# jhong93/vpd

Hardware: AMD Instinct MI355X
Metric: frame-crops/sec (VPD student train) (higher is better)
Workload: dtype bf16; 1 GPU; configs[1]: Diving48-shaped synthetic crops 128x128, ResNet-34 student (5-ch RGB+flow), emb_dim 128, sum-MSE + AdamW, batch=256 per GPU; global_batch=256, parallelism=dp1

## Files before the change

### include/vpd_hip.h

```cpp
#ifndef VPD_HIP_H
#define VPD_HIP_H
#include <stddef.h>
#ifdef __cplusplus
extern "C" {
#endif

typedef struct vpd_plan vpd_plan_t;

const char* vpd_last_error(void);
int vpd_abi_version(void);
const char* vpd_elem_dtype(void);

int vpd_plan_create(const char* arch, int c_in, int img_h, int img_w, int emb_dim, int motion,
                    int max_batch, int train, vpd_plan_t** out);
#define VPD_TRAIN_EARLY_BUCKET0 2
void vpd_plan_destroy(vpd_plan_t* plan);

int vpd_plan_num_tensors(const vpd_plan_t* plan);
int vpd_plan_tensor_info(const vpd_plan_t* plan, int i, int* kind, int* is_decoder, long long* offset,
                         long long* numel, int* ndim, int dims[4]);
long long vpd_plan_param_numel(const vpd_plan_t* plan);
int vpd_plan_num_bn(const vpd_plan_t* plan);
int vpd_plan_bn_info(const vpd_plan_t* plan, int i, int* channels, long long* rm_off, long long* rv_off);
long long vpd_plan_bn_numel(const vpd_plan_t* plan);
// ... 127 lines not shown
int vpd_graph_launch_eval(vpd_plan_t* plan, int n, void* stream);

int vpd_plan_sync_errors(vpd_plan_t* plan, void* workspace, void* stream, unsigned* count_out);

int vpd_plan_set_timing(vpd_plan_t* plan, int enable);
int vpd_plan_read_timing(vpd_plan_t* plan, double* out, int nclasses);

int vpd_op_conv2d(const void* x_bf16, const void* w_bf16, void* y_bf16, double* stats, int n, int xHp, int xWp,
                  int xC, int yHp, int yWp, int yC, int ypad, int Hs, int Ws, int osub, int oph, int opw, int istr,
                  int Kc, int Co, const int* tapset9, int accumulate, void* stream);
int vpd_op_conv_bm(int M, int Co);
int vpd_op_conv2d_ep(const void* x_bf16, const void* w_bf16, void* y_bf16, int n, int xHp, int xWp, int xC, int yHp, int yWp,
                     int yC, int ypad, int Hs, int Ws, int istr, int Kc, int Co, const int* tapset9, const float* ep_scale,
                     const float* ep_shift, const void* res_padded_bf16, int ep_relu, int accumulate,
                     const unsigned char* acc_mask, void* stream);
int vpd_op_conv2d_bnsums(const void* x_bf16, const void* w_bf16, void* y_bf16, const void* bst_z_bf16,
                         const unsigned char* bst_mask, double* rows, int n, int xHp, int xWp, int xC, int Hs, int Ws,
                         int Kc, int Co, const int* tapset9, int accumulate, void* stream);
int vpd_op_conv2d_bnsums2(const void* x_bf16, const void* w_bf16, void* y_bf16, const void* bst_z_bf16,
                          const unsigned char* bst_mask, double* rows, const void* bst_z2_bf16, double* rows2, int n, int xHp,
                          int xWp, int xC, int Hs, int Ws, int Kc, int Co, const int* tapset9, void* stream);
int vpd_op_conv2d_dispatch(int n, int xHp, int xWp, int xC, int yHp, int yWp, int yC, int ypad, int Hs, int Ws, int osub, int oph,
                           int opw, int istr, int Kc, int Co, const int* tapset9, int accumulate, int flags, int* out12);
int vpd_op_bn_forward(const void* z_bf16, const double* rows, const float* gamma, const float* beta, float* running_mean,
                      float* running_var, float* mean, float* rstd, float* scale, float* shift, const void* res_padded_bf16,
                      void* out_padded_bf16, unsigned char* mask_bits, int n, int H, int W, int C, int relu, float momentum,
                      float eps, void* stream);
int vpd_op_set_bn_frozen(int on);
int vpd_op_bn_forward2(const void* z_bf16, const double* rows, const float* gamma, const float* beta, float* running_mean,
                       float* running_var, float* mean, float* rstd, float* scale, float* shift, const void* z2_bf16,
                       const double* rows2, const float* gamma2, const float* beta2, float* running_mean2, float* running_var2,
                       float* mean2, float* rstd2, float* scale2, float* shift2, void* out_padded_bf16, unsigned char* mask_bits,
                       int n, int H, int W, int C, int relu, float momentum, float eps, void* stream);
int vpd_op_bn_finalize(double* rows, const float* gamma, const float* beta, float* running_mean, float* running_var, float* mean,
                       float* rstd, float* scale, float* shift, int count, int C, float momentum, float eps, void* stream);
int vpd_op_bn_apply(const void* z_bf16, const float* scale, const float* shift, const void* res_bf16, const float* rscale,
                    const float* rshift, int res_kind, void* out_padded_bf16, int n, int H, int W, int C, int relu, void* stream);
int vpd_op_bn_backward_apply(const void* dy_bf16, const void* z_bf16, const unsigned char* mask_bits, const double* rows,
                             const float* gamma, const float* mean, const float* rstd, void* dz_padded_bf16, float* dgamma,
                             float* dbeta, int n, int H, int W, int C, void* stream);
int vpd_op_bn_backward_apply2(const void* dy_bf16, const void* z_bf16, const unsigned char* mask_bits, const double* rows,
                              const float* gamma, const float* mean, const float* rstd, void* dz_padded_bf16, float* dgamma,
                              float* dbeta, const void* z2_bf16, const double* rows2, const float* gamma2, const float* mean2,
                              const float* rstd2, void* dz2_padded_bf16, float* dgamma2, float* dbeta2, int n, int H, int W, int C,
                              void* stream);
int vpd_op_conv1x1_bn(int mode, const void* x_padded, const void* w, int n, int H, int W, int istr, int Kc, int Co, double* rows,
// ... 76 lines not shown
```

### vpd_amd/_lib.py

```python
import ctypes as C
import os

_HERE = os.path.dirname(os.path.abspath(__file__))
LIB_PATH = os.environ.get("VPD_LIB_PATH") or os.path.join(_HERE, "libvpdhip.so")
LIB_PATH_F16 = os.environ.get("VPD_LIB_PATH_F16") or os.path.join(_HERE, "libvpdhip_f16.so")
ABI_VERSION = 5

c_int_p = C.POINTER(C.c_int)
c_ll_p = C.POINTER(C.c_longlong)
c_dbl_p = C.POINTER(C.c_double)
vp = C.c_void_p

SIGNATURES = {
    "vpd_last_error": (C.c_char_p, []),
    "vpd_abi_version": (C.c_int, []),
    "vpd_elem_dtype": (C.c_char_p, []),
    "vpd_plan_create": (C.c_int, [C.c_char_p, C.c_int, C.c_int, C.c_int, C.c_int, C.c_int, C.c_int, C.c_int,
                                  C.POINTER(vp)]),
    "vpd_plan_destroy": (None, [vp]),
    "vpd_plan_num_tensors": (C.c_int, [vp]),
    "vpd_plan_tensor_info": (C.c_int, [vp, C.c_int, c_int_p, c_int_p, c_ll_p, c_ll_p, c_int_p, c_int_p]),
    "vpd_plan_param_numel": (C.c_longlong, [vp]),
    "vpd_plan_num_bn": (C.c_int, [vp]),
    "vpd_plan_bn_info": (C.c_int, [vp, C.c_int, c_int_p, c_ll_p, c_ll_p]),
# ... 38 lines not shown
    "vpd_plan_grad_norm": (C.c_int, [vp, vp, C.c_longlong, C.c_double, vp, C.c_float, vp, vp, vp]),
    "vpd_adam_groups_bytes": (C.c_size_t, [C.c_int]),
    "vpd_adam_groups_init": (C.c_int, [vp, vp, c_ll_p, c_int_p, C.c_int, C.c_longlong, C.c_int, vp]),
    "vpd_adamw_step_groups": (C.c_int, [vp, vp, vp, vp, C.c_longlong, vp, c_dbl_p, c_dbl_p, C.c_int, C.c_double, C.c_double,
                                        C.c_double, C.c_int, C.c_float, vp, vp]),
    "vpd_plan_adamw_step_groups": (C.c_int, [vp, vp, vp, vp, vp, C.c_longlong, vp, c_dbl_p, c_dbl_p, C.c_int, C.c_double,
                                             C.c_double, C.c_double, C.c_int, vp, vp, vp]),
    "vpd_op_grad_accumulate": (C.c_int, [C.POINTER(vp), C.POINTER(vp), c_ll_p, C.c_int, C.c_int, vp]),
    "vpd_plan_grad_accum_numel": (C.c_longlong, [vp]),
    "vpd_plan_grad_accumulate": (C.c_int, [vp, vp, C.c_longlong, vp, C.c_int, vp, vp]),
    "vpd_plan_bucket_scratch_range": (C.c_int, [vp, C.c_int, C.POINTER(C.c_longlong), C.POINTER(C.c_longlong)]),
    "vpd_plan_grads_pending": (C.c_int, [vp]),
    "vpd_plan_materialize_grads": (C.c_int, [vp, vp, vp, vp]),
    "vpd_plan_set_bn_frozen": (C.c_int, [vp, C.c_int]),
    "vpd_plan_set_param_grads": (C.c_int, [vp, C.c_int]),
    "vpd_plan_set_timing": (C.c_int, [vp, C.c_int]),
    "vpd_plan_read_timing": (C.c_int, [vp, C.POINTER(C.c_double), C.c_int]),
    "vpd_op_conv2d": (C.c_int, [vp, vp, vp, vp] + [C.c_int] * 16 + [c_int_p, C.c_int, vp]),
    "vpd_op_conv_bm": (C.c_int, [C.c_int, C.c_int]),
    "vpd_op_conv2d_ep": (C.c_int, [vp, vp, vp] + [C.c_int] * 13 + [c_int_p, vp, vp, vp, C.c_int, C.c_int, vp, vp]),
    "vpd_op_conv2d_bnsums": (C.c_int, [vp] * 6 + [C.c_int] * 8 + [c_int_p, C.c_int, vp]),
    "vpd_op_conv2d_bnsums2": (C.c_int, [vp] * 8 + [C.c_int] * 8 + [c_int_p, vp]),
    "vpd_op_conv2d_dispatch": (C.c_int, [C.c_int] * 16 + [c_int_p, C.c_int, C.c_int, c_int_p]),
    "vpd_op_bn_forward": (C.c_int, [vp] * 13 + [C.c_int] * 5 + [C.c_float, C.c_float, vp]),
    "vpd_op_set_bn_frozen": (C.c_int, [C.c_int]),
    "vpd_op_bn_forward2": (C.c_int, [vp] * 22 + [C.c_int] * 5 + [C.c_float, C.c_float, vp]),
    "vpd_op_bn_finalize": (C.c_int, [vp] * 9 + [C.c_int, C.c_int, C.c_float, C.c_float, vp]),
    "vpd_op_bn_apply": (C.c_int, [vp] * 6 + [C.c_int, vp] + [C.c_int] * 5 + [vp]),
    "vpd_op_bn_backward_apply": (C.c_int, [vp] * 10 + [C.c_int] * 4 + [vp]),
    "vpd_op_bn_backward_apply2": (C.c_int, [vp] * 18 + [C.c_int] * 4 + [vp]),
    "vpd_op_conv1x1_bn": (C.c_int, [C.c_int, vp, vp] + [C.c_int] * 6 + [vp] * 5 + [C.c_float, C.c_float] + [vp] * 12),
    "vpd_op_conv1x1_bn2": (C.c_int, [C.c_int] + [vp] * 4 + [C.c_int] * 6 + [vp] * 18 + [C.c_float, C.c_float] + [vp] * 10),
    "vpd_op_conv1x1_bn_dispatch": (C.c_int, [C.c_int] * 6 + [c_int_p]),
    "vpd_op_stem_pool_forward": (C.c_int, [vp] * 5 + [C.c_int] * 5 + [vp]),
    "vpd_op_stem_dgrad": (C.c_int, [vp, vp, vp, C.c_int, C.c_int, C.c_int, C.c_int, vp]),
    "vpd_op_stem_pool_backward": (C.c_int, [vp] * 15 + [C.c_int] * 4 + [vp]),
    "vpd_op_bn_backward": (C.c_int, [vp] * 15 + [C.c_int] + [vp, vp] + [C.c_int] * 6 + [vp]),
    "vpd_op_bn_backward_pair": (C.c_int, [vp] * 20 + [C.c_int] * 4 + [vp]),
    "vpd_op_bn_backward_residency": (C.c_int, [C.c_int, C.c_int, C.c_int, c_int_p]),
    "vpd_op_avgpool": (C.c_int, [vp] + [C.c_int] * 5 + [vp, vp]),
    "vpd_op_avgpool_bwd": (C.c_int, [vp] + [C.c_int] * 4 + [vp, vp]),
    "vpd_op_sgemm": (C.c_int, [vp] * 4 + [C.c_int] * 6 + [vp]),
    "vpd_op_colsum": (C.c_int, [vp, C.c_int, C.c_int, vp, vp]),
    "vpd_op_relu_mask": (C.c_int, [vp, vp, C.c_longlong, vp]),
    "vpd_op_mse": (C.c_int, [vp, vp, C.c_longlong, vp, vp, vp, vp]),
    "vpd_op_wgrad": (C.c_int, [vp, vp, vp] + [C.c_int] * 13 + [c_int_p, vp, vp]),
# ... 71 lines not shown
```

### vpd_amd/csrc/conv_igemm.hip

```cpp
#include <stdlib.h>
#include <stdio.h>

#include <algorithm>
#include <vector>

#include "common.h"
#include "conv_epilogue.h"
#include "kernels.h"

static __device__ __forceinline__ void conv_take_alt(ConvParams& p, const ConvParams& p0, int& by) {
    if (p0.alt_w && by >= p0.alt_y0) {
        by -= p0.alt_y0;
        p.w = p0.alt_w; p.y = p0.alt_y; p.stats = p0.alt_stats; p.taps = p0.alt_taps;
        p.ep_scale = p0.alt_ep_scale; p.ep_shift = p0.alt_ep_shift; p.ep_relu = p0.alt_ep_relu; p.res = nullptr;
    }
}

static __device__ __forceinline__ int conv_pixel_base(const ConvParams& p, const ConvGeo& geo, int m) {
    const int HW = geo.Hs * geo.Ws;
    m = m < geo.M ? m : geo.M - 1;
    const int b = m / HW;
    const int r = m - b * HW;
    const int yy = r / geo.Ws;
    const int xx = r - yy * geo.Ws;
// ... 1280 lines not shown
    dim3 grid((p.M + BM - 1) / BM, p.Co / BN);
    size_t lds = ((size_t)(HALO2 ? 2 : 1) * HROWS + 2 * BN) * 64 * sizeof(bf16_t);
    const size_t red = (size_t)2 * 2 * BN * sizeof(float);
    if (lds < red) lds = red;
    ConvParams q = p;
    VPD_LAUNCH((conv3x3_halo_kernel<BM, BN, HROWS, HALO2>), grid, dim3(256), lds, stream, q, g);
    return hipGetLastError();
}

static bool halo_geom(const ConvParams& p, int BM, int hrows_max, HaloGeom* g) {
    const int W = p.Ws, H = p.Hs;
    if (BM % W != 0) return false;
    const int TR = BM / W;
    if (TR <= H) { if (H % TR != 0) return false; g->multi = 0; g->HR = TR + 2; }
    else { if (TR % H != 0) return false; g->multi = 1; g->HR = (TR / H) * (H + 2); }
    g->TR = TR;
    g->NHP = g->HR * (W + 2);
    g->total_pix = p.N * (H + 2) * (W + 2);
    if (W >= 8) { g->kmask = 7; g->kshift = 0; g->rowmask = 0; }
    else { g->kmask = 3; g->kshift = 2; g->rowmask = 1; }
    g->rH = 1.0f / (float)H; g->rW = 1.0f / (float)W; g->rWp = 1.0f / (float)(W + 2);
    g->rot = vpd_switches().pws_rot && p.Kc > 64 && conv_ep_mode(p) != 3;
    g->rnch = 1.0f / (float)(p.Kc / 64);
    return g->NHP <= hrows_max;
}

static bool halo_eligible(const ConvParams& p) {
    return p.taps.nr == 3 && p.taps.nc == 3 && p.istr == 1 && p.osub == 1 && p.oph == 0 && p.opw == 0 &&
           p.xC == p.Kc && p.xHp == p.Hs + 2 && p.xWp == p.Ws + 2 && p.taps.dy0 + 2 * p.taps.dys >= 0 &&
           p.taps.dy0 >= 0 && p.taps.dy0 <= 2 && p.taps.dx0 >= 0 && p.taps.dx0 <= 2 &&
           p.taps.dy0 + 2 * p.taps.dys <= 2 && p.taps.dx0 + 2 * p.taps.dxs >= 0 && p.taps.dx0 + 2 * p.taps.dxs <= 2;
}

template <int BM, int BN, int WM, int WN>
static hipError_t launch_cfg(const ConvParams& p, hipStream_t stream) {
    ConvParams q = p;
    const dim3 grid = conv_class_grid(q, BM, BN);
    const size_t lds = (size_t)2 * (BM + BN) * 64 * sizeof(bf16_t);
    switch (conv_ep_mode(q)) {
        case 0: VPD_LAUNCH((conv_igemm_kernel<BM, BN, WM, WN, 0>), grid, dim3(256), lds, stream, q); break;
        case 1: VPD_LAUNCH((conv_igemm_kernel<BM, BN, WM, WN, 1>), grid, dim3(256), lds, stream, q); break;
        case 2: VPD_LAUNCH((conv_igemm_kernel<BM, BN, WM, WN, 2>), grid, dim3(256), lds, stream, q); break;
        case 6: VPD_LAUNCH((conv_igemm_kernel<BM, BN, WM, WN, 6>), grid, dim3(256), lds, stream, q); break;
        case 7: VPD_LAUNCH((conv_igemm_kernel<BM, BN, WM, WN, 7>), grid, dim3(256), lds, stream, q); break;
        default: VPD_LAUNCH((conv_igemm_kernel<BM, BN, WM, WN, 3>), grid, dim3(256), lds, stream, q); break;
    }
// ... 63 lines not shown
    if (p.x2 || p.osub != 1) return false;
    if (p.yWp != p.Ws || p.yHp != p.Hs) return false;
    if (p.bst_z2) return p.accumulate && p.stats2 && (kc == 1 || kc == 2 || kc == 3 || kc == 6);
    if (kc == 0) {
        HaloGeom g2;
        return vpd_switches().dgrad_sums_l1 && !c64x2_geom(p, &g2);
    }
    return kc == 1 || kc == 2 || kc == 3 || kc == 6;
}

ConvDispatch vpd_conv_dispatch(const ConvParams& p, HaloGeom* g) {
    ConvDispatch d = {};
    d.mode = conv_ep_mode(p);
    d.kclass = vpd_conv_kernel_class(p, g);
    d.tiles_per_block = 1;
    const auto pws_form = [&](int bm, int bn, int hrows, int ns, int nmw, bool on) {
        d.bm = bm; d.bn = bn;
        d.pws = on && pws_enabled(p);
        if (!d.pws) return;
        const PwsGrid sg = pws_grid(p, bm, bn);
        d.tiles_per_block = (sg.MT + sg.lanes - 1) / sg.lanes;
        bool flip;
        d.geo = vpd_switches().pws_geo ? vpd_pws_geo_width(bm, bn, hrows, ns, nmw, p, *g, &flip) : 0;
    };
    switch (d.kclass) {
        case 0: {
            HaloGeom g2;
            d.c64x2 = c64x2_geom(p, &g2);
            if (d.c64x2) *g = g2;
            d.bm = d.c64x2 ? 256 : 128; d.bn = 64;
            const int ntiles = (p.M + d.bm - 1) / d.bm;
            int per;
            const int grid = persistent_grid(ntiles, &per);
            d.tiles_per_block = (ntiles + grid - 1) / grid;
            return d;
        }
        case 1: pws_form(256, 128, 352, PWS_NS_C1, 8, (p.M + 255) / 256 > pws_cu_count() / (p.Co / 128)); return d;
        case 2: pws_form(128, 128, 288, PWS_NS_C2, 4, true); return d;
        case 3: pws_form(128, 64, 288, PWS_NS_C3, 4, true); return d;
        case 6: pws_form(256, 64, 416, PWS_NS_C6, 4, true); return d;
        case 5: {
            d.bm = 128; d.bn = 64;
            const int grid = stem_grid(p);
            d.tiles_per_block = p.pool_y ? (p.N + grid - 1) / grid * (p.Hs * p.Ws / 128) : (p.M / 128 + grid - 1) / grid;
            return d;
        }
// ... 64 lines not shown
```

### vpd_amd/csrc/conv_pws.h

```cpp
#pragma once
#include <type_traits>

#include "common.h"
#include "conv_epilogue.h"

struct HaloGeom {
    int TR;
    int multi;
    int HR;
    int NHP;
    int total_pix;
    int kmask, kshift, rowmask;
    float rH, rW, rWp;
    int rot;
    float rnch;
};

typedef const void __attribute__((address_space(1)))* gptr_t;
typedef void __attribute__((address_space(3)))* lptr_t;

int pws_cu_count();
#ifndef PWS_NS_C1
#define PWS_NS_C1 4
#endif
#ifndef PWS_NS_C2
#define PWS_NS_C2 5
#endif
#ifndef PWS_NS_C3
#define PWS_NS_C3 9
#endif
#ifndef PWS_NS_C6
#define PWS_NS_C6 5
#endif

int vpd_conv_kernel_class(const ConvParams& p, HaloGeom* g);

struct PwsGrid {
    int lanes;
// ... 99 lines not shown
                yoff = ((size_t)(bi * p.yHp + yy * p.osub + geo.oph + p.ypad) * p.yWp + (xx * p.osub + geo.opw + p.ypad)) * p.yC;
            }
            const size_t e = yoff + n0 + wn * WTN;
            const bf16_t* t0 = ACC ? p.y : p.bst_z;
            const bf16_t* t1 = (BSTM && ZTOO) ? p.bst_z : t0;
            const bf16_t* t2 = EPM == 8 ? p.bst_z2 : t1;
            const unsigned char* mk = BSTM ? p.bst_mask : p.acc_mask;
            src = fq == 0 ? (const void*)(t0 + e) : fq == 1 ? (const void*)(t1 + e) : (const void*)(t2 + e);
            if (fq == 3 && mk && (BSTM ? ZTOO : true)) src = (const void*)((size_t)(mk + (e >> 3)) & ~(size_t)15);
        }
        pws_dma16(src, dump);
    }
}

template <int W_PER, int HPASS, int HT, int A>
struct PwsSched {
    static constexpr int cnt(int t) { return t < HT ? HPASS / HT + (t < HPASS % HT ? 1 : 0) : 0; }
    static constexpr int first(int t) { int k = 0; for (int v = 0; v < t; ++v) k += cnt(v); return k; }
    static constexpr int per(int t) { return W_PER + cnt(t); }
    static constexpr int inflight(int t) { int n = 0; for (int k = 1; k < A; ++k) n += per(((t - k) % 9 + 9) % 9); return n; }
    static constexpr int max_inflight() { int m = 0; for (int t = 0; t < 9; ++t) m = inflight(t) > m ? inflight(t) : m; return m; }
};

template <int BM, int BN, int HROWS, int NS, int EPM, int NMW, bool PIPE, int WC = 0, bool FLIP = false>
static __device__ __forceinline__ void pws_body(const ConvParams& p, const HaloGeom& g, const PwsGrid& sg) {
    constexpr int WN = BN / 64;
    constexpr int WM = NMW / WN;
    constexpr int WTM = BM / WM;
    constexpr int MI = WTM / 16, NI = 4;
    constexpr int WSTAGE = BN * 64;
    constexpr int HBUF = HROWS * 64;
    constexpr int W_PER = BN / 32;
    constexpr int HINSTR = HROWS / 8;
    constexpr int HPASS = (HINSTR + 3) / 4;
    constexpr int A = NS - 2;
    constexpr int HT = 9 - A;
    using SC = PwsSched<W_PER, HPASS, HT, A>;
    static_assert(HROWS % 8 == 0 && A >= 1 && HT >= 1 && SC::max_inflight() < 64, "ring / vmcnt geometry");
    static_assert(EPM == 0 || EPM == 1 || EPM == 2 || EPM == 3 || EPM == 6 || EPM == 7 || EPM == 8, "epilogue mode");
    static_assert(WC == 0 || NMW == 4 || NMW == 8, "compile-time geometry: four or eight MFMA waves (always the two-set fragment pipeline)");
    constexpr unsigned OFF_W = 2u * HBUF * 2u;
    constexpr unsigned OFF_DUMP = OFF_W + NS * WSTAGE * 2u;
    constexpr unsigned OFF_RED = OFF_DUMP + 1024u;

    extern __shared__ __attribute__((aligned(16))) unsigned char smem[];
    unsigned char* red = smem + OFF_RED;
    pws_kernarg_touch<sizeof(ConvParams) + sizeof(HaloGeom) + sizeof(PwsGrid)>();

    const ConvGeo geo = {p.Hs, p.Ws, p.M, p.oph, p.opw};
    const int tid = threadIdx.x;
    const int lane = tid & 63;
    const int wave = __builtin_amdgcn_readfirstlane(tid >> 6);
    const int W = p.Ws, H = p.Hs, Wp = W + 2;
    const int Ci = p.Kc;
    const int nchunks = Ci >> 6;
    const int nsteps = nchunks * 9;

    PWS_STAMP(wave == 0 ? 0 : 8);
    int lane0, nt;
    {
        const int b = blockIdx.x;
        const float rNT = sg.rNT;
        if (sg.xcd) { const int k = b >> 3; const int q = vpd_fdiv(k, rNT); nt = k - q * sg.NT; lane0 = q * 8 + (b & 7); }
        else { lane0 = vpd_fdiv(b, rNT); nt = b - lane0 * sg.NT; }
    }
    const int n0 = nt * BN;
    const int njobs = lane0 < sg.MT ? vpd_fdiv(sg.MT - lane0 + sg.lanes - 1, sg.rlanes) : 0;
    if (njobs == 0) return;
    const int total = njobs * nsteps;
    const unsigned lds0 = (unsigned)(size_t)(lptr_t)smem;

    if (wave >= NMW) {
#ifdef PWS_LOADER_PRIO
        __builtin_amdgcn_s_setprio(PWS_LOADER_PRIO);
#endif
        const int lw = wave - NMW;
        const int piece = lane & 7;
        const int lrow = lane >> 3;
        unsigned hoff[HPASS];
        auto halo_off = [&](int k) __attribute__((always_inline)) {
            const int hp = (lw + 4 * k) * 8 + lrow;
            const int hr = vpd_fdiv(hp, g.rWp);
            const int key = ((hp - hr * Wp) & g.kmask) ^ ((hr & g.rowmask) << g.kshift);
            return (unsigned)(hp * Ci * 2 + ((piece ^ key) << 4));
        };
        auto tile_gp0 = [&](int mtile) __attribute__((always_inline)) {
            const int gr0 = mtile * g.TR;
            const int b = vpd_fdiv(gr0, g.rH);
            const int prow0 = g.multi ? b * (H + 2) : b * (H + 2) + (gr0 - b * H);
            return __builtin_amdgcn_readfirstlane(prow0 * Wp);
        };
        auto tile_rot = [&](int mtile) __attribute__((always_inline)) {
            if (!g.rot) return 0;
            return __builtin_amdgcn_readfirstlane(mtile - vpd_fdiv(mtile, g.rnch) * nchunks);
        };
        auto effcc = [&](int cc, int r) __attribute__((always_inline)) { const int e = cc + r; return e >= nchunks ? e - nchunks : e; };
        auto halo_instr = [&](int gp0, int cc, int buf, int k) __attribute__((always_inline)) {
            if (HINSTR % 4 != 0 && lw + 4 * k >= HINSTR) { pws_dma16(p.w, lds0 + OFF_DUMP); return; }
            const unsigned dst = lds0 + (unsigned)buf * (HBUF * 2u) + (unsigned)(lw + 4 * k) * 1024u;
            if (gp0 + HINSTR * 8 <= g.total_pix) {
                pws_dma16s(reinterpret_cast<const char*>(p.x) + ((size_t)gp0 * Ci + cc * 64) * 2, hoff[k], dst);
            } else {
                const int hp = (lw + 4 * k) * 8 + lrow;
                const int gp = gp0 + hp < g.total_pix ? gp0 + hp : g.total_pix - 1;
                const unsigned swz = (hoff[k] - (unsigned)(hp * Ci * 2)) >> 1;
                pws_dma16(p.x + (size_t)gp * Ci + cc * 64 + swz, dst);
            }
        };
        unsigned wrow[W_PER];
#pragma unroll
        for (int i = 0; i < W_PER; ++i) {
            const int n = (lw + 4 * i) * 8 + lrow;
            wrow[i] = (unsigned)(((n0 + n) * Ci + ((piece ^ (n & 7)) << 3)) * 2);
        }
        auto issue_w = [&](int tap, int cc, unsigned stg) __attribute__((always_inline)) {
            const int wsl = p.taps.w0 + (tap / 3) * p.taps.wrs + (tap % 3) * p.taps.wcs;
            const char* wbp = reinterpret_cast<const char*>(p.w) + ((size_t)wsl * p.Co * Ci + cc * 64) * 2;
#pragma unroll
            for (int k = 0; k < W_PER; ++k)
                pws_dma16s(wbp, wrow[k], lds0 + OFF_W + stg * (WSTAGE * 2u) + (unsigned)(lw + 4 * k) * 1024u);
        };
        int w_job = 0, wrot = tile_rot(lane0);
        {
            const int gp0 = tile_gp0(lane0);
            PWS_STAMP(12);
#pragma unroll
// ... 34 lines not shown
                if constexpr (SC::cnt(t) > 0) {
                    if (has_next && !VPD_ABL(p, 4)) {
#pragma unroll
                        for (int u = 0; u < SC::cnt(t); ++u) halo_instr(h_gp0, h_cce, h_buf, SC::first(t) + u);
                    }
                }
            };
            step(std::integral_constant<int, 0>{}); step(std::integral_constant<int, 1>{}); step(std::integral_constant<int, 2>{});
            step(std::integral_constant<int, 3>{}); step(std::integral_constant<int, 4>{}); step(std::integral_constant<int, 5>{});
            step(std::integral_constant<int, 6>{}); step(std::integral_constant<int, 7>{}); step(std::integral_constant<int, 8>{});
            if (++h_cc == nchunks) { h_cc = 0; ++h_job; hrot = tile_rot(lane0 + h_job * sg.lanes); }
        }
        pws_vmwait<0>();
        PWS_STAMP(11);
        PWS_STAMP_RT(15);
        __builtin_amdgcn_s_barrier();
        return;
    }

    const int wm = wave % WM;
    const int wn = wave / WM;
    const int fr = lane & 15;
    const int fq = lane >> 4;
    unsigned lo[3][MI];
    {
        const float rW = g.rW, rH = g.rH;
#pragma unroll
        for (int b = 0; b < MI; ++b) {
            const int m = wm * WTM + b * 16 + fr;
            const int lr = vpd_fdiv(m, rW);
            const int xx = m - lr * W;
            const int li = vpd_fdiv(lr, rH);
            const int hrow = g.multi ? li * (H + 2) + (lr - li * H) : lr;
            const unsigned rowkey = (unsigned)(((hrow & g.rowmask) << g.kshift) ^ fq);
#pragma unroll
            for (int ic = 0; ic < 3; ++ic)
                lo[ic][b] = (unsigned)((hrow * Wp + xx) * 128) +
                            ((((unsigned)(xx + p.taps.dx0 + ic * p.taps.dxs) & (unsigned)g.kmask) ^ rowkey) << 4);
        }
    }
    unsigned wa0;
    {
        const int r = wn * 64 + fr;
        wa0 = (unsigned)(r * 128 + ((fq ^ (r & 7)) << 4));
    }
    constexpr bool BST = EPM == 6 || EPM == 7 || EPM == 8;
// ... 280 lines not shown
            const int c = tid - which * BN;
            const int rmask = (p.stat_rows ? p.stat_rows : VPD_STAT_ROWS) - 1;
            if (p.stats) {
                float t = 0.f;
#pragma unroll
                for (int w = 0; w < WM; ++w) t += redf[(w * 3 + which) * BN + c];
                atomicAdd(&p.stats[((size_t)(blockIdx.x & rmask) * 2 + which) * p.Co + n0 + c], (double)t);
            }
            if (EPM == 8 && p.stats2) {
                float t = 0.f;
#pragma unroll
                for (int w = 0; w < WM; ++w) t += redf[(w * 3 + (which ? 2 : 0)) * BN + c];
                atomicAdd(&p.stats2[((size_t)(blockIdx.x & rmask) * 2 + which) * p.Co + n0 + c], (double)t);
            }
        }
    }
    PWS_STAMP(6);
#ifdef PWS_STAMPS
    asm volatile("s_waitcnt vmcnt(0)" ::: "memory");
    PWS_STAMP(7);
#endif
}

template <int BM, int BN, int HROWS, int NS, int EPM, int NMW, bool PIPE, int WC = 0, bool FLIP = false>
__global__ __launch_bounds__((NMW + 4) * 64, (NMW + 4) / 4) void conv3x3_pws_kernel(const ConvParams p, const HaloGeom g,
                                                                                   const PwsGrid sg) {
    pws_body<BM, BN, HROWS, NS, EPM, NMW, PIPE, WC, FLIP>(p, g, sg);
}

bool vpd_launch_pws_geo(int bm, int bn, int hrows, int ns, int nmw, const ConvParams& q, const HaloGeom& g, const PwsGrid& sg, dim3 grid,
                        dim3 block, size_t lds, hipStream_t stream);
int vpd_pws_geo_width(int bm, int bn, int hrows, int ns, int nmw, const ConvParams& q, const HaloGeom& g, bool* flip_out);
```

### vpd_amd/csrc/conv_pws_geo.hip

```cpp
#include <hip/hip_runtime.h>

#include "conv_pws.h"
#include "kernels.h"

namespace {

template <int BM, int BN, int HROWS, int NS, int WC, int NMW = 4, bool PIPE = true>
bool launch_geo(bool flip, const ConvParams& q, const HaloGeom& g, const PwsGrid& sg, dim3 grid, dim3 block, size_t lds,
                hipStream_t stream) {
    const int mode = conv_ep_mode(q);
    if (!flip) {
        switch (mode) {
            case 1: VPD_LAUNCH((conv3x3_pws_kernel<BM, BN, HROWS, NS, 1, NMW, PIPE, WC, false>), grid, block, lds, stream, q, g, sg); return true;
            case 3: VPD_LAUNCH((conv3x3_pws_kernel<BM, BN, HROWS, NS, 3, NMW, PIPE, WC, false>), grid, block, lds, stream, q, g, sg); return true;
            default: return false;
        }
    }
    switch (mode) {
        case 0: VPD_LAUNCH((conv3x3_pws_kernel<BM, BN, HROWS, NS, 0, NMW, PIPE, WC, true>), grid, block, lds, stream, q, g, sg); return true;
        case 2: VPD_LAUNCH((conv3x3_pws_kernel<BM, BN, HROWS, NS, 2, NMW, PIPE, WC, true>), grid, block, lds, stream, q, g, sg); return true;
        case 6: VPD_LAUNCH((conv3x3_pws_kernel<BM, BN, HROWS, NS, 6, NMW, PIPE, WC, true>), grid, block, lds, stream, q, g, sg); return true;
        case 7: VPD_LAUNCH((conv3x3_pws_kernel<BM, BN, HROWS, NS, 7, NMW, PIPE, WC, true>), grid, block, lds, stream, q, g, sg); return true;
        case 8: VPD_LAUNCH((conv3x3_pws_kernel<BM, BN, HROWS, NS, 8, NMW, PIPE, WC, true>), grid, block, lds, stream, q, g, sg); return true;
        default: return false;
    }
}

}

int vpd_pws_geo_width(int bm, int bn, int hrows, int ns, int nmw, const ConvParams& q, const HaloGeom& g, bool* flip_out) {
    const TapSet& t = q.taps;
    const bool fwd = t.dy0 == 0 && t.dys == 1 && t.dx0 == 0 && t.dxs == 1;
    const bool flip = t.dy0 == 2 && t.dys == -1 && t.dx0 == 2 && t.dxs == -1;
    if (!fwd && !flip) return 0;
    if (q.Ws >= 8 ? !(g.kmask == 7 && g.kshift == 0 && g.rowmask == 0) : !(g.kmask == 3 && g.kshift == 2 && g.rowmask == 1)) return 0;
    const int mode = conv_ep_mode(q);
    if (flip ? !(mode == 0 || mode == 2 || mode == 6 || mode == 7 || mode == 8) : !(mode == 1 || mode == 3)) return 0;
    *flip_out = flip;
    if (nmw == 4 && bm == 256 && bn == 64 && hrows == 416 && ns == PWS_NS_C6) return q.Ws == 16 || q.Ws == 8 ? q.Ws : 0;
    if (nmw == 4 && bm == 128 && bn == 64 && hrows == 288 && ns == PWS_NS_C3) return q.Ws == 4 ? 4 : 0;
    return 0;
}

bool vpd_launch_pws_geo(int bm, int bn, int hrows, int ns, int nmw, const ConvParams& q, const HaloGeom& g, const PwsGrid& sg, dim3 grid,
                        dim3 block, size_t lds, hipStream_t stream) {
    bool flip = false;
    switch (vpd_pws_geo_width(bm, bn, hrows, ns, nmw, q, g, &flip)) {
        case 16: return launch_geo<256, 64, 416, PWS_NS_C6, 16>(flip, q, g, sg, grid, block, lds, stream);
        case 8: return launch_geo<256, 64, 416, PWS_NS_C6, 8>(flip, q, g, sg, grid, block, lds, stream);
        case 4: return launch_geo<128, 64, 288, PWS_NS_C3, 4>(flip, q, g, sg, grid, block, lds, stream);
        default: return false;
    }
}
```

### vpd_amd/csrc/kernels.h

```cpp
#pragma once
#include <string.h>

#include <vector>

#include "common.h"

struct BnApplyParams {
    const bf16_t* z;
    const float* scale; const float* shift;
    int res_kind;
    const bf16_t* res; int rHp, rWp, rpad;
    const float* rscale; const float* rshift;
    bf16_t* out; int oHp, oWp, opad;
    int M, H, W, C, relu;
    unsigned char* mask_out;
    int xcd_tile_px;
};

struct StemPoolParams {
    const bf16_t* z; int Hz, Wz;
    const float* scale; const float* shift;
    bf16_t* out; int opad;
    unsigned char* idx;
    int N, Ho, Wo, C;
// ... 45 lines not shown
}
struct AdamGroupHyper { AdamHyper h; const void* table; float decay[VPD_MAX_PARAM_GROUPS], step_size[VPD_MAX_PARAM_GROUPS]; };
struct AdamGroupHyperDyn { AdamGroupHyper g; const vpd_scale_state* st; double lr[VPD_MAX_PARAM_GROUPS], b1, b2; };
struct AdamGroupArgs { const void* table; const double* lr; const double* wd; int ngroups; double b1, b2, eps; int step; float gscale;
                       const vpd_scale_state* st; };
#define FR_MAX 96
struct FiniteRanges {
    const float* ptr[FR_MAX];
    long n[FR_MAX];
    int count;
};

hipError_t vpd_launch_conv(const ConvParams& p, hipStream_t stream);
hipError_t vpd_launch_scale(float* x, long n, float s, hipStream_t stream);
bool vpd_conv1x1_stream_eligible(const ConvParams& p);
hipError_t vpd_launch_conv1x1_stream(const ConvParams& p, hipStream_t stream);
void vpd_conv1x1_stream_grid(const ConvParams& p, int* bm, int* bn, int* lanes);
int vpd_conv_kernel_class(const ConvParams& p);
bool vpd_conv_takes_bn_sums(const ConvParams& p);
struct ConvDispatch {
    int kclass;
    int pws;
    int geo;
    int c64x2;
    int ws1x1, stream1x1;
    int halo;
    int bm, bn;
    int mode;
    int tiles_per_block;
};
ConvDispatch vpd_conv_dispatch(const ConvParams& p);
int vpd_conv_xcd_tile_px(const ConvParams& p);
hipError_t vpd_launch_wgrad_reduce(const WgradParams& p, hipStream_t stream);
extern "C" int vpd_conv_bm(int M, int Co);
hipError_t vpd_launch_wgrad(const WgradParams& p, hipStream_t stream);
size_t vpd_wgrad_slab_bytes();
bool vpd_wgrad_group_eligible(const WgradParams& p);
size_t vpd_wgrad_group_slab_floats(int M, int Co, int Kc, int ntaps = 9);
hipError_t vpd_launch_wgrad_group(const WgradParams* ps, int n, hipStream_t stream);
bool vpd_wgrad_overwrites(const WgradParams& p);
bool vpd_wgrad_dispatch(const WgradParams& p, int* out9);
int vpd_wgrad_group_dispatch(const WgradParams* ps, int n, int* head4, int* per3);
int vpd_wgrad_group_max();
bool vpd_wgrad_pair_ok(const WgradParams& p3, const WgradParams& p1);
hipError_t vpd_launch_wgrad_pair(const WgradParams& p3, const WgradParams& p1, hipStream_t stream);
hipError_t vpd_launch_wgrad_pair_reduce(const WgradParams& p3, const WgradParams& p1, hipStream_t stream);
// ... 202 lines not shown
```

### vpd_amd/csrc/ops.hip

```cpp
#include <hip/hip_runtime.h>
#include <string.h>

#include <vector>

#include "plan.h"

static int g_op_bn_frozen = 0;
extern "C" int vpd_op_set_bn_frozen(int on) { g_op_bn_frozen = on != 0; return 0; }

extern "C" int vpd_op_conv_bm(int M, int Co) { return vpd_conv_bm(M, Co); }
extern "C" size_t vpd_op_wgrad_slab_bytes(void) { return vpd_wgrad_slab_bytes(); }

static TapSet tapset_from(const int* t) {
    TapSet ts;
    ts.nr = t[0]; ts.nc = t[1]; ts.dy0 = t[2]; ts.dys = t[3]; ts.dx0 = t[4]; ts.dxs = t[5];
    ts.w0 = t[6]; ts.wrs = t[7]; ts.wcs = t[8];
    return ts;
}
static ConvParams op_conv_params(const void* x, const void* w, void* y, int n, int xHp, int xWp, int xC, int yHp, int yWp, int yC,
                                 int ypad, int Hs, int Ws, int istr, int Kc, int Co, const int* tapset9) {
    ConvParams q = vpd_conv_params((const bf16_t*)x, xHp, xWp, xC, (const bf16_t*)w, n, Hs, Ws, istr, Kc, Co, tapset_from(tapset9));
    q.y = (bf16_t*)y; q.yHp = yHp; q.yWp = yWp; q.yC = yC; q.ypad = ypad;
    return q;
}
// ... 53 lines not shown
    ConvParams q = op_conv_params(x, w, y, n, xHp, xWp, xC, Hs, Ws, Co, 0, Hs, Ws, 1, Kc, Co, tapset9);
    q.accumulate = accumulate;
    q.bst_z = (const bf16_t*)bst_z; q.bst_mask = bst_mask; vpd_conv_set_bn_rows(q, rows);
    q.bst_z2 = (const bf16_t*)bst_z2; q.stats2 = rows2;
    if (q.taps.nr < 1 || q.taps.nc < 1) return fail("empty tap set");
    if (!vpd_conv_takes_bn_sums(q)) return fail("no kernel takes the BatchNorm sums for this shape");
    LCHECK(vpd_launch_conv(q, (hipStream_t)stream));
    return 0;
}

extern "C" int vpd_op_conv2d_bnsums(const void* x, const void* w, void* y, const void* bst_z, const unsigned char* bst_mask,
                                    double* rows, int n, int xHp, int xWp, int xC, int Hs, int Ws, int Kc, int Co,
                                    const int* tapset9, int accumulate, void* stream) {
    return op_conv2d_bnsums(x, w, y, bst_z, bst_mask, rows, nullptr, nullptr, n, xHp, xWp, xC, Hs, Ws, Kc, Co, tapset9, accumulate, stream);
}

extern "C" int vpd_op_conv2d_bnsums2(const void* x, const void* w, void* y, const void* bst_z, const unsigned char* bst_mask,
                                     double* rows, const void* bst_z2, double* rows2, int n, int xHp, int xWp, int xC, int Hs,
                                     int Ws, int Kc, int Co, const int* tapset9, void* stream) {
    if (!bst_z2 || !rows2) return fail("null argument");
    return op_conv2d_bnsums(x, w, y, bst_z, bst_mask, rows, bst_z2, rows2, n, xHp, xWp, xC, Hs, Ws, Kc, Co, tapset9, 1, stream);
}

extern "C" int vpd_op_conv2d_dispatch(int n, int xHp, int xWp, int xC, int yHp, int yWp, int yC, int ypad, int Hs, int Ws, int osub,
                                      int oph, int opw, int istr, int Kc, int Co, const int* tapset9, int accumulate, int flags,
                                      int* out12) {
    if (!tapset9 || !out12) return fail("null argument");
    if (n < 1 || Hs < 1 || Ws < 1 || xHp < 1 || xWp < 1 || xC < 1 || yC < Co || Kc < 64 || Kc % 64 || Co < 64 || Co % 64 || osub < 1 ||
        istr < 1 || (long long)n * Hs * Ws >= (1ll << 31) || (flags & ~31))
        return fail("bad argument");
    if ((flags & 16) && !(flags & 8)) return fail("a second BatchNorm needs the first");
    static const double present = 0.0;
    ConvParams q = op_conv_params(nullptr, nullptr, nullptr, n, xHp, xWp, xC, yHp, yWp, yC, ypad, Hs, Ws, istr, Kc, Co, tapset9);
    q.osub = osub; q.oph = oph; q.opw = opw; q.accumulate = accumulate;
    if (flags & 1) q.stats = const_cast<double*>(&present);
    if (flags & 2) { q.ep_scale = (const float*)&present; q.ep_shift = (const float*)&present; }
    if (flags & 4) q.acc_mask = (const unsigned char*)&present;
    if (flags & 8) { q.bst_z = (const bf16_t*)&present; q.bst_mask = (const unsigned char*)&present; vpd_conv_set_bn_rows(q, const_cast<double*>(&present)); }
    if (flags & 16) { q.bst_z2 = (const bf16_t*)&present; q.stats2 = const_cast<double*>(&present); }
    if (q.taps.nr < 1 || q.taps.nc < 1) return fail("empty tap set");
    const ConvDispatch d = vpd_conv_dispatch(q);
    const int v[12] = {d.kclass, d.pws, d.geo, d.c64x2, d.ws1x1, d.stream1x1, d.halo, d.bm, d.bn, d.mode, d.tiles_per_block,
                       (flags & 8) ? (int)vpd_conv_takes_bn_sums(q) : 0};
    memcpy(out12, v, sizeof v);
    return 0;
}

extern "C" int vpd_op_bn_forward(const void* z, const double* rows, const float* gamma, const float* beta, float* running_mean,
                                 float* running_var, float* mean, float* rstd, float* scale, float* shift, const void* res,
                                 void* out, unsigned char* mask_bits, int n, int H, int W, int C, int relu, float momentum,
                                 float eps, void* stream) {
    if (!z || !rows || !gamma || !beta || !mean || !rstd || !scale || !shift || !out) return fail("null argument");
    if (n < 1 || H < 1 || W < 1 || C < 8 || C % 8 || C > 4096) return fail("bad shape");
    BnApplyParams a = vpd_bn_apply_params((const bf16_t*)z, res ? 1 : 0, (const bf16_t*)res, (bf16_t*)out, n, H, W, C, relu);
    a.mask_out = mask_bits;
    const BnFusedFwd f = op_fused_fwd(op_fwd_side(rows, gamma, beta, running_mean, running_var, mean, rstd, scale, shift), a.M, momentum, eps);
    if (f.frozen && (!running_mean || !running_var)) return fail("a frozen BatchNorm needs running_mean and running_var");
    LCHECK(vpd_launch_bn_fwd_fused(a, f, (hipStream_t)stream));
    return 0;
}

extern "C" int vpd_op_bn_forward2(const void* z, const double* rows, const float* gamma, const float* beta, float* running_mean,
                                  float* running_var, float* mean, float* rstd, float* scale, float* shift, const void* z2,
                                  const double* rows2, const float* gamma2, const float* beta2, float* running_mean2,
                                  float* running_var2, float* mean2, float* rstd2, float* scale2, float* shift2, void* out,
                                  unsigned char* mask_bits, int n, int H, int W, int C, int relu, float momentum, float eps,
                                  void* stream) {
// ... 596 lines not shown
```

### vpd_amd/csrc/switches.h

```cpp
#pragma once
#include <stdlib.h>

#define VPD_SWITCHES(X)                                        \
    X(fused_bn,           "VPD_FUSED_BN",          1)          \
    X(bn_pair,            "VPD_BN_PAIR",           1)          \
    X(bn_xcd,             "VPD_BN_XCD",            1)          \
    X(bn_xcd_force,       "VPD_BN_XCD_FORCE",     -1)          \
    X(dgrad_sums,         "VPD_DGRAD_SUMS",        1)          \
    X(dgrad_sums_l1,      "VPD_DGRAD_SUMS_L1",     1)          \
    X(dgrad_sums_s2,      "VPD_DGRAD_SUMS_S2",     1)          \
    X(dgrad_sums_pair,    "VPD_DGRAD_SUMS_PAIR",   1)          \
    X(dgrad_sums_1x1,     "VPD_DGRAD_SUMS_1X1",    1)          \
    X(relu_bits,          "VPD_RELU_BITS",         1)          \
    X(poolbwd_fold,       "VPD_POOLBWD_FOLD",      1)          \
    X(ds_merge,           "VPD_DS_MERGE",          1)          \
    X(pws,                "VPD_PWS",               1)          \
    X(pws_blocks,         "VPD_PWS_BLOCKS",        0)          \
    X(ws_256x64,          "VPD_WS_256x64",         1)          \
    X(ws_mw8,             "VPD_WS_MW8",            1)          \
    X(no_ws,              "VPD_NO_WS",             0)          \
    X(pws_geo,            "VPD_PWS_GEO",           1)          \
    X(pws_rot,            "VPD_PWS_ROT",           1)          \
    X(reserve_cus,        "VPD_RESERVE_CUS",       0)          \
    X(c64x2,              "VPD_C64X2",             1)          \
    X(conv1x1_ws,         "VPD_CONV1X1_WS",        1)          \
    X(conv_s2_ws,         "VPD_CONV_S2_WS",        1)          \
    X(conv_s2_dgrad_ws,   "VPD_CONV_S2_DGRAD_WS",  1)          \
    X(wg2,                "VPD_WG2",               1)          \
    X(wg2_1x1,            "VPD_WG2_1X1",           1)          \
    X(wg2_tco256,         "VPD_WG2_TCO256",        1)          \
    X(conv1x1_stream,     "VPD_CONV1X1_STREAM",    1)          \
    X(bneck_recompute,    "VPD_BNECK_RECOMPUTE",   1)          \
    X(wg_group,           "VPD_WG_GROUP",          1)          \
    X(wg_merge,           "VPD_WG_MERGE",          1)          \
    X(wgrad_1x1,          "VPD_WGRAD_1X1",        -1)          \
    X(wgrad_s2,           "VPD_WGRAD_S2",          1)          \
    X(wgrad_ds_ride,      "VPD_WGRAD_DS_RIDE",     1)          \
    X(stem_lds_store,     "VPD_STEM_LDS_STORE",    1)          \
    X(stem_pair,          "VPD_STEM_PAIR",         1)          \
    X(stem_quad,          "VPD_STEM_QUAD",         1)          \
    X(stem_poolsums,      "VPD_STEM_POOLSUMS",     1)          \
    X(stem_pool_fused,    "VPD_STEM_POOL_FUSED",   1)          \
    X(ablate,             "VPD_ABLATE",            0)

struct VpdSwitches {
// ... 16 lines not shown
```

Baseline: 78380 crops/s.

## Load only interior halo pixels in geometry-specialized PWS conv and zero borders in LDS

Adds an interior mode to the compile-time-width PWS 3x3 conv kernel. When the tile covers whole images, the halo DMA fetches only the interior rows and columns of each padded image. The zero padding border is written directly into both LDS halo buffers once at kernel start. This cuts global loads of padding pixels and drops the filler instruction, but adds per-block LDS zeroing, more template instantiations and a new dispatch query entry point.

```diff
diff --git a/include/vpd_hip.h b/include/vpd_hip.h
--- a/include/vpd_hip.h
+++ b/include/vpd_hip.h
@@ -173,6 +173,8 @@
                           int xWp, int xC, int Hs, int Ws, int Kc, int Co, const int* tapset9, void* stream);
 int vpd_op_conv2d_dispatch(int n, int xHp, int xWp, int xC, int yHp, int yWp, int yC, int ypad, int Hs, int Ws, int osub, int oph,
                            int opw, int istr, int Kc, int Co, const int* tapset9, int accumulate, int flags, int* out12);
+int vpd_op_conv2d_interior(int n, int xHp, int xWp, int xC, int yHp, int yWp, int yC, int ypad, int Hs, int Ws, int osub, int oph,
+                           int opw, int istr, int Kc, int Co, const int* tapset9, int accumulate, int flags, int* out);
 int vpd_op_bn_forward(const void* z_bf16, const double* rows, const float* gamma, const float* beta, float* running_mean,
                       float* running_var, float* mean, float* rstd, float* scale, float* shift, const void* res_padded_bf16,
                       void* out_padded_bf16, unsigned char* mask_bits, int n, int H, int W, int C, int relu, float momentum,
diff --git a/vpd_amd/_lib.py b/vpd_amd/_lib.py
--- a/vpd_amd/_lib.py
+++ b/vpd_amd/_lib.py
@@ -84,6 +84,7 @@
     "vpd_op_conv2d_bnsums": (C.c_int, [vp] * 6 + [C.c_int] * 8 + [c_int_p, C.c_int, vp]),
     "vpd_op_conv2d_bnsums2": (C.c_int, [vp] * 8 + [C.c_int] * 8 + [c_int_p, vp]),
     "vpd_op_conv2d_dispatch": (C.c_int, [C.c_int] * 16 + [c_int_p, C.c_int, C.c_int, c_int_p]),
+    "vpd_op_conv2d_interior": (C.c_int, [C.c_int] * 16 + [c_int_p, C.c_int, C.c_int, c_int_p]),
     "vpd_op_bn_forward": (C.c_int, [vp] * 13 + [C.c_int] * 5 + [C.c_float, C.c_float, vp]),
     "vpd_op_set_bn_frozen": (C.c_int, [C.c_int]),
     "vpd_op_bn_forward2": (C.c_int, [vp] * 22 + [C.c_int] * 5 + [C.c_float, C.c_float, vp]),
diff --git a/vpd_amd/csrc/conv_igemm.hip b/vpd_amd/csrc/conv_igemm.hip
--- a/vpd_amd/csrc/conv_igemm.hip
+++ b/vpd_amd/csrc/conv_igemm.hip
@@ -1326,6 +1326,8 @@
     g->rH = 1.0f / (float)H; g->rW = 1.0f / (float)W; g->rWp = 1.0f / (float)(W + 2);
     g->rot = vpd_switches().pws_rot && p.Kc > 64 && conv_ep_mode(p) != 3;
     g->rnch = 1.0f / (float)(p.Kc / 64);
+    g->interior = 0;
+    g->rHp = 1.0f / (float)(H + 2);
     return g->NHP <= hrows_max;
 }
 
@@ -1435,6 +1437,8 @@
         d.tiles_per_block = (sg.MT + sg.lanes - 1) / sg.lanes;
         bool flip;
         d.geo = vpd_switches().pws_geo ? vpd_pws_geo_width(bm, bn, hrows, ns, nmw, p, *g, &flip) : 0;
+        g->interior = vpd_switches().pws_interior && d.geo && (bm / p.Ws) % p.Hs == 0 && (p.Ws != 4 || p.Hs == 4);
+        d.interior = g->interior;
     };
     switch (d.kclass) {
         case 0: {
diff --git a/vpd_amd/csrc/conv_pws.h b/vpd_amd/csrc/conv_pws.h
--- a/vpd_amd/csrc/conv_pws.h
+++ b/vpd_amd/csrc/conv_pws.h
@@ -14,6 +14,8 @@
     float rH, rW, rWp;
     int rot;
     float rnch;
+    int interior;
+    float rHp;
 };
 
 typedef const void __attribute__((address_space(1)))* gptr_t;
@@ -159,7 +161,7 @@
     static constexpr int max_inflight() { int m = 0; for (int t = 0; t < 9; ++t) m = inflight(t) > m ? inflight(t) : m; return m; }
 };
 
-template <int BM, int BN, int HROWS, int NS, int EPM, int NMW, bool PIPE, int WC = 0, bool FLIP = false>
+template <int BM, int BN, int HROWS, int NS, int EPM, int NMW, bool PIPE, int WC = 0, bool FLIP = false, bool INT = false>
 static __device__ __forceinline__ void pws_body(const ConvParams& p, const HaloGeom& g, const PwsGrid& sg) {
     constexpr int WN = BN / 64;
     constexpr int WM = NMW / WN;
@@ -168,7 +170,7 @@
     constexpr int WSTAGE = BN * 64;
     constexpr int HBUF = HROWS * 64;
     constexpr int W_PER = BN / 32;
-    constexpr int HINSTR = HROWS / 8;
+    constexpr int HINSTR = !INT ? HROWS / 8 : WC == 4 ? BM / 16 * 3 : BM / 8;
     constexpr int HPASS = (HINSTR + 3) / 4;
     constexpr int A = NS - 2;
     constexpr int HT = 9 - A;
@@ -176,6 +178,7 @@
     static_assert(HROWS % 8 == 0 && A >= 1 && HT >= 1 && SC::max_inflight() < 64, "ring / vmcnt geometry");
     static_assert(EPM == 0 || EPM == 1 || EPM == 2 || EPM == 3 || EPM == 6 || EPM == 7 || EPM == 8, "epilogue mode");
     static_assert(WC == 0 || NMW == 4 || NMW == 8, "compile-time geometry: four or eight MFMA waves (always the two-set fragment pipeline)");
+    static_assert(!INT || ((WC == 16 || WC == 8 || WC == 4) && HINSTR % 4 == 0), "interior mode: compile-time width, no filler instruction");
     constexpr unsigned OFF_W = 2u * HBUF * 2u;
     constexpr unsigned OFF_DUMP = OFF_W + NS * WSTAGE * 2u;
     constexpr unsigned OFF_RED = OFF_DUMP + 1024u;
@@ -215,8 +218,21 @@
         const int piece = lane & 7;
         const int lrow = lane >> 3;
         unsigned hoff[HPASS];
+        int hbase[INT ? HPASS : 1];
+        auto halo_pix0 = [&](int k) __attribute__((always_inline)) {
+            const int j = lw + 4 * k;
+            if constexpr (!INT) return j * 8;
+            else if constexpr (WC == 4) { const int img = j / 3; return img * 36 + 7 + (j - img * 3) * 8; }
+            else {
+                const int r = WC == 16 ? j >> 1 : j;
+                const int img = vpd_fdiv(r, g.rH);
+                return __builtin_amdgcn_readfirstlane((img * (H + 2) + (r - img * H) + 1) * Wp + 1 + (WC == 16 ? (j & 1) * 8 : 0));
+            }
+        };
         auto halo_off = [&](int k) __attribute__((always_inline)) {
-            const int hp = (lw + 4 * k) * 8 + lrow;
+            const int hp0 = halo_pix0(k);
+            if constexpr (INT) hbase[k] = hp0;
+            const int hp = hp0 + lrow;
             const int hr = vpd_fdiv(hp, g.rWp);
             const int key = ((hp - hr * Wp) & g.kmask) ^ ((hr & g.rowmask) << g.kshift);
             return (unsigned)(hp * Ci * 2 + ((piece ^ key) << 4));
@@ -234,11 +250,12 @@
         auto effcc = [&](int cc, int r) __attribute__((always_inline)) { const int e = cc + r; return e >= nchunks ? e - nchunks : e; };
         auto halo_instr = [&](int gp0, int cc, int buf, int k) __attribute__((always_inline)) {
             if (HINSTR % 4 != 0 && lw + 4 * k >= HINSTR) { pws_dma16(p.w, lds0 + OFF_DUMP); return; }
-            const unsigned dst = lds0 + (unsigned)buf * (HBUF * 2u) + (unsigned)(lw + 4 * k) * 1024u;
-            if (gp0 + HINSTR * 8 <= g.total_pix) {
+            const int hp0 = INT ? hbase[k] : (lw + 4 * k) * 8;
+            const unsigned dst = lds0 + (unsigned)buf * (HBUF * 2u) + (unsigned)hp0 * 128u;
+            if (gp0 + (INT ? g.NHP : HINSTR * 8) <= g.total_pix) {
                 pws_dma16s(reinterpret_cast<const char*>(p.x) + ((size_t)gp0 * Ci + cc * 64) * 2, hoff[k], dst);
             } else {
-                const int hp = (lw + 4 * k) * 8 + lrow;
+                const int hp = hp0 + lrow;
                 const int gp = gp0 + hp < g.total_pix ? gp0 + hp : g.total_pix - 1;
                 const unsigned swz = (hoff[k] - (unsigned)(hp * Ci * 2)) >> 1;
                 pws_dma16(p.x + (size_t)gp * Ci + cc * 64 + swz, dst);
@@ -319,6 +336,31 @@
     const int wn = wave / WM;
     const int fr = lane & 15;
     const int fq = lane >> 4;
+    if constexpr (INT) {
+        constexpr int Wpc = WC + 2;
+        typedef unsigned u32x4_t __attribute__((ext_vector_type(4)));
+        typedef u32x4_t __attribute__((address_space(3)))* lds16_t;
+        const u32x4_t zero = {0u, 0u, 0u, 0u};
+        const float rHp = g.rHp;
+        static_assert(!INT || HROWS * 8 % (NMW * 64) == 0, "interior mode: whole passes over a halo buffer");
+#pragma unroll
+        for (int it = 0; it < HROWS * 8 / (NMW * 64); ++it) {
+            const int i = tid + it * (NMW * 64);
+            const int hp = i >> 3;
+            int border;
+            if constexpr (WC == 4) { const int q = hp % 36; border = (q < 7) | (q > 30); }
+            else {
+                const int hr = hp / Wpc, xp = hp - hr * Wpc;
+                const int ri = hr - vpd_fdiv(hr, rHp) * (H + 2);
+                border = (xp == 0) | (xp == Wpc - 1) | (ri == 0) | (ri == H + 1);
+            }
+            if (border | (hp >= g.NHP)) {
+                *(lds16_t)(size_t)(lds0 + (unsigned)i * 16u) = zero;
+                *(lds16_t)(size_t)(lds0 + HBUF * 2u + (unsigned)i * 16u) = zero;
+            }
+        }
+        asm volatile("s_waitcnt lgkmcnt(0)" ::: "memory");
+    }
     unsigned lo[3][MI];
     {
         const float rW = g.rW, rH = g.rH;
@@ -645,10 +687,10 @@
 #endif
 }
 
-template <int BM, int BN, int HROWS, int NS, int EPM, int NMW, bool PIPE, int WC = 0, bool FLIP = false>
+template <int BM, int BN, int HROWS, int NS, int EPM, int NMW, bool PIPE, int WC = 0, bool FLIP = false, bool INT = false>
 __global__ __launch_bounds__((NMW + 4) * 64, (NMW + 4) / 4) void conv3x3_pws_kernel(const ConvParams p, const HaloGeom g,
                                                                                    const PwsGrid sg) {
-    pws_body<BM, BN, HROWS, NS, EPM, NMW, PIPE, WC, FLIP>(p, g, sg);
+    pws_body<BM, BN, HROWS, NS, EPM, NMW, PIPE, WC, FLIP, INT>(p, g, sg);
 }
 
 bool vpd_launch_pws_geo(int bm, int bn, int hrows, int ns, int nmw, const ConvParams& q, const HaloGeom& g, const PwsGrid& sg, dim3 grid,
diff --git a/vpd_amd/csrc/conv_pws_geo.hip b/vpd_amd/csrc/conv_pws_geo.hip
--- a/vpd_amd/csrc/conv_pws_geo.hip
+++ b/vpd_amd/csrc/conv_pws_geo.hip
@@ -5,23 +5,23 @@
 
 namespace {
 
-template <int BM, int BN, int HROWS, int NS, int WC, int NMW = 4, bool PIPE = true>
+template <int BM, int BN, int HROWS, int NS, int WC, bool INT, int NMW = 4, bool PIPE = true>
 bool launch_geo(bool flip, const ConvParams& q, const HaloGeom& g, const PwsGrid& sg, dim3 grid, dim3 block, size_t lds,
                 hipStream_t stream) {
     const int mode = conv_ep_mode(q);
     if (!flip) {
         switch (mode) {
-            case 1: VPD_LAUNCH((conv3x3_pws_kernel<BM, BN, HROWS, NS, 1, NMW, PIPE, WC, false>), grid, block, lds, stream, q, g, sg); return true;
-            case 3: VPD_LAUNCH((conv3x3_pws_kernel<BM, BN, HROWS, NS, 3, NMW, PIPE, WC, false>), grid, block, lds, stream, q, g, sg); return true;
+            case 1: VPD_LAUNCH((conv3x3_pws_kernel<BM, BN, HROWS, NS, 1, NMW, PIPE, WC, false, INT>), grid, block, lds, stream, q, g, sg); return true;
+            case 3: VPD_LAUNCH((conv3x3_pws_kernel<BM, BN, HROWS, NS, 3, NMW, PIPE, WC, false, INT>), grid, block, lds, stream, q, g, sg); return true;
             default: return false;
         }
     }
     switch (mode) {
-        case 0: VPD_LAUNCH((conv3x3_pws_kernel<BM, BN, HROWS, NS, 0, NMW, PIPE, WC, true>), grid, block, lds, stream, q, g, sg); return true;
-        case 2: VPD_LAUNCH((conv3x3_pws_kernel<BM, BN, HROWS, NS, 2, NMW, PIPE, WC, true>), grid, block, lds, stream, q, g, sg); return true;
-        case 6: VPD_LAUNCH((conv3x3_pws_kernel<BM, BN, HROWS, NS, 6, NMW, PIPE, WC, true>), grid, block, lds, stream, q, g, sg); return true;
-        case 7: VPD_LAUNCH((conv3x3_pws_kernel<BM, BN, HROWS, NS, 7, NMW, PIPE, WC, true>), grid, block, lds, stream, q, g, sg); return true;
-        case 8: VPD_LAUNCH((conv3x3_pws_kernel<BM, BN, HROWS, NS, 8, NMW, PIPE, WC, true>), grid, block, lds, stream, q, g, sg); return true;
+        case 0: VPD_LAUNCH((conv3x3_pws_kernel<BM, BN, HROWS, NS, 0, NMW, PIPE, WC, true, INT>), grid, block, lds, stream, q, g, sg); return true;
+        case 2: VPD_LAUNCH((conv3x3_pws_kernel<BM, BN, HROWS, NS, 2, NMW, PIPE, WC, true, INT>), grid, block, lds, stream, q, g, sg); return true;
+        case 6: VPD_LAUNCH((conv3x3_pws_kernel<BM, BN, HROWS, NS, 6, NMW, PIPE, WC, true, INT>), grid, block, lds, stream, q, g, sg); return true;
+        case 7: VPD_LAUNCH((conv3x3_pws_kernel<BM, BN, HROWS, NS, 7, NMW, PIPE, WC, true, INT>), grid, block, lds, stream, q, g, sg); return true;
+        case 8: VPD_LAUNCH((conv3x3_pws_kernel<BM, BN, HROWS, NS, 8, NMW, PIPE, WC, true, INT>), grid, block, lds, stream, q, g, sg); return true;
         default: return false;
     }
 }
@@ -45,10 +45,17 @@
 bool vpd_launch_pws_geo(int bm, int bn, int hrows, int ns, int nmw, const ConvParams& q, const HaloGeom& g, const PwsGrid& sg, dim3 grid,
                         dim3 block, size_t lds, hipStream_t stream) {
     bool flip = false;
-    switch (vpd_pws_geo_width(bm, bn, hrows, ns, nmw, q, g, &flip)) {
-        case 16: return launch_geo<256, 64, 416, PWS_NS_C6, 16>(flip, q, g, sg, grid, block, lds, stream);
-        case 8: return launch_geo<256, 64, 416, PWS_NS_C6, 8>(flip, q, g, sg, grid, block, lds, stream);
-        case 4: return launch_geo<128, 64, 288, PWS_NS_C3, 4>(flip, q, g, sg, grid, block, lds, stream);
+    const int wc = vpd_pws_geo_width(bm, bn, hrows, ns, nmw, q, g, &flip);
+    if (g.interior) switch (wc) {
+        case 16: return launch_geo<256, 64, 416, PWS_NS_C6, 16, true>(flip, q, g, sg, grid, block, lds, stream);
+        case 8: return launch_geo<256, 64, 416, PWS_NS_C6, 8, true>(flip, q, g, sg, grid, block, lds, stream);
+        case 4: return launch_geo<128, 64, 288, PWS_NS_C3, 4, true>(flip, q, g, sg, grid, block, lds, stream);
+        default: return false;
+    }
+    switch (wc) {
+        case 16: return launch_geo<256, 64, 416, PWS_NS_C6, 16, false>(flip, q, g, sg, grid, block, lds, stream);
+        case 8: return launch_geo<256, 64, 416, PWS_NS_C6, 8, false>(flip, q, g, sg, grid, block, lds, stream);
+        case 4: return launch_geo<128, 64, 288, PWS_NS_C3, 4, false>(flip, q, g, sg, grid, block, lds, stream);
         default: return false;
     }
 }
diff --git a/vpd_amd/csrc/kernels.h b/vpd_amd/csrc/kernels.h
--- a/vpd_amd/csrc/kernels.h
+++ b/vpd_amd/csrc/kernels.h
@@ -91,6 +91,7 @@
     int kclass;
     int pws;
     int geo;
+    int interior;
     int c64x2;
     int ws1x1, stream1x1;
     int halo;
diff --git a/vpd_amd/csrc/ops.hip b/vpd_amd/csrc/ops.hip
--- a/vpd_amd/csrc/ops.hip
+++ b/vpd_amd/csrc/ops.hip
@@ -99,10 +99,8 @@
     return op_conv2d_bnsums(x, w, y, bst_z, bst_mask, rows, bst_z2, rows2, n, xHp, xWp, xC, Hs, Ws, Kc, Co, tapset9, 1, stream);
 }
 
-extern "C" int vpd_op_conv2d_dispatch(int n, int xHp, int xWp, int xC, int yHp, int yWp, int yC, int ypad, int Hs, int Ws, int osub,
-                                      int oph, int opw, int istr, int Kc, int Co, const int* tapset9, int accumulate, int flags,
-                                      int* out12) {
-    if (!tapset9 || !out12) return fail("null argument");
+static int op_conv2d_dispatch(int n, int xHp, int xWp, int xC, int yHp, int yWp, int yC, int ypad, int Hs, int Ws, int osub, int oph, int opw,
+                              int istr, int Kc, int Co, const int* tapset9, int accumulate, int flags, ConvDispatch* d, int* takes_sums) {
     if (n < 1 || Hs < 1 || Ws < 1 || xHp < 1 || xWp < 1 || xC < 1 || yC < Co || Kc < 64 || Kc % 64 || Co < 64 || Co % 64 || osub < 1 ||
         istr < 1 || (long long)n * Hs * Ws >= (1ll << 31) || (flags & ~31))
         return fail("bad argument");
@@ -116,10 +114,31 @@
     if (flags & 8) { q.bst_z = (const bf16_t*)&present; q.bst_mask = (const unsigned char*)&present; vpd_conv_set_bn_rows(q, const_cast<double*>(&present)); }
     if (flags & 16) { q.bst_z2 = (const bf16_t*)&present; q.stats2 = const_cast<double*>(&present); }
     if (q.taps.nr < 1 || q.taps.nc < 1) return fail("empty tap set");
-    const ConvDispatch d = vpd_conv_dispatch(q);
-    const int v[12] = {d.kclass, d.pws, d.geo, d.c64x2, d.ws1x1, d.stream1x1, d.halo, d.bm, d.bn, d.mode, d.tiles_per_block,
-                       (flags & 8) ? (int)vpd_conv_takes_bn_sums(q) : 0};
+    *d = vpd_conv_dispatch(q);
+    *takes_sums = (flags & 8) ? (int)vpd_conv_takes_bn_sums(q) : 0;
+    return 0;
+}
+extern "C" int vpd_op_conv2d_dispatch(int n, int xHp, int xWp, int xC, int yHp, int yWp, int yC, int ypad, int Hs, int Ws, int osub,
+                                      int oph, int opw, int istr, int Kc, int Co, const int* tapset9, int accumulate, int flags,
+                                      int* out12) {
+    if (!tapset9 || !out12) return fail("null argument");
+    ConvDispatch d;
+    int sums;
+    const int rc = op_conv2d_dispatch(n, xHp, xWp, xC, yHp, yWp, yC, ypad, Hs, Ws, osub, oph, opw, istr, Kc, Co, tapset9, accumulate, flags, &d, &sums);
+    if (rc) return rc;
+    const int v[12] = {d.kclass, d.pws, d.geo, d.c64x2, d.ws1x1, d.stream1x1, d.halo, d.bm, d.bn, d.mode, d.tiles_per_block, sums};
     memcpy(out12, v, sizeof v);
+    return 0;
+}
+extern "C" int vpd_op_conv2d_interior(int n, int xHp, int xWp, int xC, int yHp, int yWp, int yC, int ypad, int Hs, int Ws, int osub,
+                                      int oph, int opw, int istr, int Kc, int Co, const int* tapset9, int accumulate, int flags,
+                                      int* out) {
+    if (!tapset9 || !out) return fail("null argument");
+    ConvDispatch d;
+    int sums;
+    const int rc = op_conv2d_dispatch(n, xHp, xWp, xC, yHp, yWp, yC, ypad, Hs, Ws, osub, oph, opw, istr, Kc, Co, tapset9, accumulate, flags, &d, &sums);
+    if (rc) return rc;
+    *out = d.interior;
     return 0;
 }
 
diff --git a/vpd_amd/csrc/switches.h b/vpd_amd/csrc/switches.h
--- a/vpd_amd/csrc/switches.h
+++ b/vpd_amd/csrc/switches.h
@@ -21,6 +21,7 @@
     X(no_ws,              "VPD_NO_WS",             0)          \
     X(pws_geo,            "VPD_PWS_GEO",           1)          \
     X(pws_rot,            "VPD_PWS_ROT",           1)          \
+    X(pws_interior,       "VPD_PWS_INTERIOR",      1)          \
     X(reserve_cus,        "VPD_RESERVE_CUS",       0)          \
     X(c64x2,              "VPD_C64X2",             1)          \
     X(conv1x1_ws,         "VPD_CONV1X1_WS",        1)          \
```

New measurement: 79470 crops/s, median of 6. 1.01x the previous value.
